# sortmerna/sortmerna

Hardware: NVIDIA H100
Metric: reads/sec (150 bp vs SILVA-8) (higher is better)
Workload: dtype int16x2 (DPX) / u8

## Files before the change

### include/smr_b200.h

```cpp
#ifndef SMR_B200_H
#define SMR_B200_H
#include <stddef.h>
#include <stdint.h>

#ifdef __cplusplus
extern "C" {
#endif

typedef struct smr_ctx smr_ctx;

enum smr_status {
  SMR_OK = 0,
  SMR_ERR_CUDA = 1,
  SMR_ERR_ARG = 2,
  SMR_ERR_INDEX = 3,
  SMR_ERR_UNSUPPORTED = 4,
  SMR_ERR_CAPACITY = 5,
  SMR_ERR_NO_DEVICE = 6
};

typedef struct {
  int32_t match, mismatch, score_N, gap_open, gap_ext;
  int32_t num_seeds, min_lis, edges, edges_is_percent;
  int32_t num_alignments, is_best;
// ... 106 lines not shown
  int32_t out2, sout;
} smr_report_opts;

int smr_format_reports(smr_ctx*, const smr_report_opts* opts, const char* text, uint64_t nbytes, const smr_read_result* results,
                       const smr_aln* alns, const uint32_t* cigar_pool, uint64_t cigar_words, const smr_aln_stats* stats, uint32_t nreads,
                       char* out, uint64_t cap, uint64_t* stream_off);
int smr_format_reports_gz(smr_ctx*, const smr_report_opts* opts, const char* text, uint64_t nbytes, const smr_read_result* results,
                          const smr_aln* alns, const uint32_t* cigar_pool, uint64_t cigar_words, const smr_aln_stats* stats, uint32_t nreads,
                          char* out, uint64_t cap, uint64_t* stream_off);
int smr_gzip(smr_ctx*, const void* in, uint64_t n, void* out, uint64_t cap, uint64_t* out_bytes);
int smr_last_report_timings(const smr_ctx*, double out[3]);

typedef struct {
  double min_id, min_cov;
  int32_t paired_in, paired_out;
} smr_otu_opts;
int smr_otu_begin(smr_ctx*, const smr_otu_opts* opts);
int smr_otu_add(smr_ctx*, const char* text, uint64_t nbytes, const smr_read_result* results, const smr_aln* alns, const smr_aln_stats* stats,
                uint32_t nreads, uint64_t* n_added);
int smr_otu_finish(smr_ctx*, char* out, uint64_t cap, uint64_t counts[3]);
int smr_last_otu_timings(const smr_ctx*, double out[3]);

int smr_last_timings(const smr_ctx*, double out[8]);


int smr_debug_seed_windows(smr_ctx*, uint32_t part_slot, const uint8_t* seq_cat, const uint64_t* seq_off,
                           uint32_t nreads, const uint32_t* win_read, const uint32_t* win_pos, uint32_t nwin,
                           uint32_t* ids, uint32_t cap, uint32_t* counts, uint8_t* zero);
int smr_debug_dpx_peak(smr_ctx*, double* giga_ops_per_s);
int smr_debug_ssw(smr_ctx*, const uint8_t* q_cat, const uint64_t* q_off, const uint8_t* t_cat,
                  const uint64_t* t_off, uint32_t npairs, uint32_t filters, int32_t* out, uint32_t* cigars,
                  uint32_t cigar_cap);

#ifdef __cplusplus
}
#endif
#endif
```

### sortmerna_b200/api.py

```python
from __future__ import annotations

import ctypes as C
import os

import numpy as np

from . import hostio

HERE = os.path.dirname(os.path.abspath(__file__))
LIB_PATH = os.environ.get("SMR_LIB_PATH") or os.path.join(HERE, "libsmr_b200.so")

STATUS = {0: "SMR_OK", 1: "SMR_ERR_CUDA", 2: "SMR_ERR_ARG", 3: "SMR_ERR_INDEX", 4: "SMR_ERR_UNSUPPORTED",
          5: "SMR_ERR_CAPACITY", 6: "SMR_ERR_NO_DEVICE"}

SYMBOLS = ["smr_init", "smr_destroy", "smr_last_error", "smr_device_count", "smr_load_index_part",
           "smr_set_minimal_score", "smr_set_params", "smr_index_info", "smr_align_batch", "smr_upload_batch",
           "smr_run_resident", "smr_download_results", "smr_last_timings", "smr_debug_seed_windows", "smr_debug_ssw",
           "smr_debug_dpx_peak", "smr_set_stats_buffer", "smr_build_index", "smr_upload_fastx", "smr_resident_layout", "smr_pack_kvdb_blobs",
           "smr_set_aln_slots", "smr_aln_slots", "smr_aln_slots_needed", "smr_upload_fastx_gz", "smr_resident_text", "smr_debug_inflate",
           "smr_build_index_device", "smr_debug_index_array", "smr_set_instrumentation", "smr_set_report_refs", "smr_set_report_scoring",
           "smr_format_reports", "smr_last_report_timings", "smr_otu_begin", "smr_otu_add", "smr_otu_finish", "smr_last_otu_timings",
           "smr_format_reports_gz", "smr_gzip"]

CNT_NAMES = ("num_aligned", "num_short", "sw_calls", "sw_cells", "windows", "trie_nodes", "buckets",
             "bucket_entries", "pos_entries", "lis_calls", "dbg_max_read_cycles", "dbg_sum_read_cycles", "dbg_lis_kernel_cycles",
             "cyc_vote", "cyc_order", "cyc_group", "cyc_plan", "cyc_wait", "cyc_replay", "spec_calls", "spec_cells", "spec_pairs", "slow_pairs",
             "sc_wait", "sc_load", "sc_sw", "sc_pub", "rounds_a", "rounds_b", "w1_cyc", "w1_cnt", "dbg_max_read_busy_cycles")
CNT_FIXED = 32


class Params(C.Structure):
    _fields_ = [(n, C.c_int32) for n in (
        "match", "mismatch", "score_N", "gap_open", "gap_ext", "num_seeds", "min_lis", "edges",
        "edges_is_percent", "num_alignments", "is_best", "is_forward", "is_reverse", "is_full_search",
        "minoccur")]


def default_params(**kw) -> Params:
    p = Params(match=2, mismatch=-3, score_N=-3, gap_open=5, gap_ext=2, num_seeds=2, min_lis=2, edges=4,
               edges_is_percent=0, num_alignments=1, is_best=1, is_forward=1, is_reverse=1, is_full_search=0,
               minoccur=0)
    for k, v in kw.items():
        setattr(p, k, v)
    return p

# ... 395 lines not shown
        rc = self.L.smr_otu_finish(self.h, _ptr(buf), C.c_uint64(buf.size), _ptr(counts))
        if rc == 5 and int(counts[0]) > buf.size:
            buf = np.zeros(int(counts[0]) + (int(counts[0]) >> 3), np.uint8)
            rc = self.L.smr_otu_finish(self.h, _ptr(buf), C.c_uint64(buf.size), _ptr(counts))
        self._check(rc, "smr_otu_finish")
        self._otu_buf = buf
        return dict(text=bytes(buf[:int(counts[0])]), total_otu=int(counts[1]), n_yid_ycov=int(counts[2]))

    def otu_timings(self):
        out = np.zeros(3, np.float64)
        self._check(self.L.smr_last_otu_timings(self.h, _ptr(out)), "smr_last_otu_timings")
        return dict(add_h2d_ms=out[0], add_device_ms=out[1], finish_ms=out[2])

    def report_timings(self):
        out = np.zeros(3, np.float64)
        self._check(self.L.smr_last_report_timings(self.h, _ptr(out)), "smr_last_report_timings")
        return dict(h2d_ms=out[0], device_ms=out[1], d2h_ms=out[2])

    def timings(self):
        out = np.zeros(8, np.float64)
        self.L.smr_last_timings(self.h, _ptr(out))
        return dict(total_ms=out[0], seed_ms=out[1], lis_ms=out[2], final_ms=out[3], h2d_ms=out[4], d2h_ms=out[5],
                    launches=int(out[6]), decode_ms=out[7])

    def dpx_peak(self) -> float:
        v = C.c_double(0)
        self._check(self.L.smr_debug_dpx_peak(self.h, C.byref(v)), "smr_debug_dpx_peak")
        return v.value

    def debug_seed_windows(self, part_slot, cat03, off, win_read, win_pos, cap=64, fallback_path=False):
        cat03 = np.ascontiguousarray(cat03, np.uint8)
        off = np.ascontiguousarray(off, np.uint64)
        win_read = np.ascontiguousarray(win_read, np.uint32)
        win_pos = np.ascontiguousarray(win_pos, np.uint32)
        nwin = win_read.size
        ids = np.zeros(nwin * cap, np.uint32)
        counts = np.zeros(nwin, np.uint32)
        zero = np.zeros(nwin, np.uint8)
        rc = self.L.smr_debug_seed_windows(self.h, C.c_uint32(part_slot), _ptr(cat03), _ptr(off), C.c_uint32(off.size - 1),
                                           _ptr(win_read), _ptr(win_pos), C.c_uint32(nwin), _ptr(ids),
                                           C.c_uint32(cap | (0x80000000 if fallback_path else 0)), _ptr(counts), _ptr(zero))
        self._check(rc, "smr_debug_seed_windows")
        return ids.reshape(nwin, cap), counts, zero

    def debug_ssw(self, q_cat, q_off, t_cat, t_off, filters=0, cigar_cap=256):
        q_cat = np.ascontiguousarray(q_cat, np.uint8)
# ... 93 lines not shown
```

### sortmerna_b200/csrc/smr_capi.cu

```cuda
#include "../../include/smr_b200.h"

#include <algorithm>
#include <cmath>
#include <cstdio>
#include <cstdlib>
#include <cstring>
#include <mutex>
#include <string>
#include <thread>
#include <vector>

#include "smr_decode.cuh"
#include "smr_report.cuh"
#include "smr_otu.cuh"
#include "smr_inflate.cuh"
#include "smr_deflate.cuh"
#include "smr_build.h"
#include "smr_build_dev.cuh"
#include "smr_final.cuh"
#include "smr_index.h"

using namespace smr;

namespace {
// ... 42 lines not shown
  uint32_t need_slots = 0;
  uint32_t all_slots = 16;
  uint32_t lis_ctas_per_sm = kLisMinCtas;

  uint32_t nreads = 0; uint64_t total_nt = 0; uint32_t max_len = 0;
  std::vector<uint8_t> h_seq; std::vector<uint64_t> h_off;
  std::vector<uint32_t> off32;
  DevBuf seq04, seq_off, pk03, pk03alt, pk_off, has_n, hit_cnt, flags, state, hit_db, aln_work, out_aln;
  DevBuf hits, cost, bins, scalars, counters, cigar_pool, parts_dev;
  size_t hits_stride = 0; uint32_t cnt_stride = 0;
  DevBuf lis_arena, lis_epochs, lis_queue, lis_done, lis_rows, lis_dbg, final_arena, lane_hits, tb_arena, tb_jobs, fin_list, aln_stats;
  smr_aln_stats* host_stats = nullptr;
  PinBuf h_state, h_flags, h_hitdb, h_outaln, h_stats, h_cigar, h_off32, h_pkoff;
  std::vector<uint64_t> h_coff;
  DevBuf d_text, d_hdroff;
  DevBuf d_cnt, d_scal, d_nl, d_hdr, d_sb, d_rec, d_spos;
  DevBuf cub_tmp;
  DevBuf seed_ctr, d_gz, d_cand, d_res, d_sym, d_win, d_ids, d_off, d_cnt64, d_moff, d_mem, d_poff, d_plen, d_pcrc;
  uint64_t text_bytes = 0;
  uint32_t inf_spans = 0, inf_candidates = 0; double t_inflate = 0;
  bool device_only_reads = false;
  double t_decode = 0;
  uint32_t tb_threads = 0, tb_cap_w = 0, tb_cap_cig = 0; size_t tb_cap_dir = 0, tb_stride = 0;
  uint32_t lis_warps = 0, final_warps = 0;
  size_t lis_stride = 0, final_stride = 0;
  uint32_t hist_cap = 0, cand_cap = 0, pair_cap = 0, row_cap = 0, pall_cap = 0, task_cap = 0, cap_w = 0, cap_cig = 0; size_t cap_dir = 0;
  uint32_t lis_ctas = 0;
  uint32_t lane_hits_cap = 0, lane_hits_warps = 0;
  uint64_t cigar_cap_dev = 0;
  uint32_t scale = 1;
  bool instr = false;
  uint64_t flag_hist[6] = {0, 0, 0, 0, 0, 0};
  struct RptScore { bool set = false; DevBuf ev, bits; };
  std::vector<RptScore> rpt_score;
  DevBuf r_text, r_line, r_recs, r_res, r_aln, r_cig, r_st, r_flags, r_keys, r_keys2, r_vals, r_rows, r_first,
         r_sz, r_off, r_bsz, r_boff, r_fxsz, r_fxoff, r_grp, r_so, r_out;
  double t_rpt[3] = {0, 0, 0};
  DevBuf z_in, z_chunk, z_m, z_freq, z_codes, z_hdr, z_info, z_scratch, z_poff, z_plen, z_crc, z_dst, z_trl, z_out;
  uint64_t parts_gen = 0;
  struct Otu {
    bool active = false; uint64_t gen = 0; double min_id = 0, min_cov = 0;
    std::vector<RptGroup> groups; uint32_t gbits = 0, kbits = 0;
    DevBuf rank, rank_off, grp, key, ent, pool, flag, pos, nsz, noff, vals, skey, sidx, size, off, out, scal;
    uint64_t n = 0, pool_bytes = 0;
    double t[3] = {0, 0, 0};
  } otu;
// ... 155 lines not shown
  pt.d.flookup = p_flookup; pt.d.ftext = p_ftext; pt.d.fid = p_fid; pt.d.pos_off = p_posoff; pt.d.pos = p_pos;
  pt.d.refseq = p_ref; pt.d.ref_off = p_roff;
  pt.n_entries = E; pt.n_ids = nids; pt.n_pos = npos; pt.n_refseq = c04.size();
  return SMR_OK;
}

DevParams to_dev(const smr_params& p) {
  DevParams d;
  d.match = p.match; d.mismatch = p.mismatch; d.score_N = p.score_N; d.gap_open = p.gap_open; d.gap_ext = p.gap_ext;
  d.num_seeds = p.num_seeds; d.min_lis = p.min_lis; d.edges = p.edges; d.edges_is_percent = p.edges_is_percent;
  d.num_alignments = p.num_alignments; d.is_best = p.is_best; d.is_forward = p.is_forward; d.is_reverse = p.is_reverse;
  d.is_full_search = p.is_full_search;
  d.one = 1;
  return d;
}

uint32_t pow2_ge(uint32_t v) { uint32_t p = 1; while (p < v) p <<= 1; return p; }

cudaEvent_t get_event(smr_ctx* ctx, size_t i) {
  while (ctx->ev.size() <= i) { cudaEvent_t e; cudaEventCreate(&e); ctx->ev.push_back(e); }
  return ctx->ev[i];
}

struct Scalars { uint32_t* work_n; uint32_t* lis_next; uint32_t* fin_next; uint32_t* lis_next_b; unsigned long long* cigar_used; uint32_t* fin_jobs; uint32_t* q_head; uint32_t* q_tail; uint32_t* planners_done; };
Scalars scalars_of(smr_ctx* ctx) {
  uint8_t* p = (uint8_t*)ctx->scalars.p;
  return Scalars{(uint32_t*)p, (uint32_t*)(p + 4), (uint32_t*)(p + 8), (uint32_t*)(p + 12), (unsigned long long*)(p + 16), (uint32_t*)(p + 24), (uint32_t*)(p + 128), (uint32_t*)(p + 256), (uint32_t*)(p + 384)};
}

int setup_arenas(smr_ctx* ctx) {
  uint32_t max_nref = 1;
  for (auto& pt : ctx->parts) max_nref = std::max(max_nref, pt.d.nref);
  ctx->hist_cap = max_nref;
  ctx->cand_cap = std::max(64u, max_nref);
  ctx->pair_cap = pow2_ge(4096u * ctx->scale);
  ctx->task_cap = 2 * ctx->pair_cap;
  const uint32_t edges = ctx->prm.edges_is_percent ? (uint32_t)((ctx->prm.edges / 100.0) * (double)ctx->max_len) : (uint32_t)std::max(0, ctx->prm.edges);
  ctx->row_cap = ctx->max_len + 2 * edges + 2 * 64 + 64;
  int occ = 0;
  CK(cudaFuncSetAttribute(lis_kernel<false>, cudaFuncAttributeMaxDynamicSharedMemorySize, kLisSmemBytes));
  CK(cudaFuncSetAttribute(lis_kernel<true>, cudaFuncAttributeMaxDynamicSharedMemorySize, kLisSmemBytes));
  CK(cudaOccupancyMaxActiveBlocksPerMultiprocessor(&occ, lis_kernel<true>, kLisWarpsPerCta * 32, kLisSmemBytes));
  if (occ < 1) { ctx->err = "lis_kernel does not fit on an SM"; return SMR_ERR_CUDA; }
  ctx->lis_ctas = (uint32_t)ctx->sm_count * std::min<uint32_t>(ctx->lis_ctas_per_sm, (uint32_t)occ);
  ctx->lis_warps = ctx->lis_ctas * kPlannerWarps;
  ctx->pall_cap = 32768u * ctx->scale;
  ctx->lis_stride = lis_arena_bytes(ctx->hist_cap, ctx->cand_cap, ctx->pair_cap, ctx->task_cap, ctx->pall_cap);
  const size_t budget = (size_t)16 << 30;
  while (ctx->lis_ctas > 16 && ctx->lis_stride * ctx->lis_warps > budget) { ctx->lis_ctas /= 2; ctx->lis_warps = ctx->lis_ctas * kPlannerWarps; }
  if (int rc = ensure(ctx, ctx->lis_arena, ctx->lis_stride * ctx->lis_warps)) return rc;
  if (int rc = ensure(ctx, ctx->lis_epochs, (size_t)ctx->lis_warps * 4)) return rc;
  if (int rc = ensure(ctx, ctx->lis_queue, (size_t)2 * kQueueCap * sizeof(QSlot) + 64)) return rc;
  if (int rc = ensure(ctx, ctx->lis_done, (size_t)ctx->lis_warps * 4 + 64)) return rc;
  const size_t dbg_bytes = (size_t)(kTlBase + kTlRows * kTlBuckets) * 8;
  if (int rc = ensure(ctx, ctx->lis_dbg, dbg_bytes)) return rc;
  CK(cudaMemsetAsync(ctx->lis_dbg.p, 0, dbg_bytes, ctx->stream));
  if (int rc = ensure(ctx, ctx->lis_rows, (size_t)ctx->lis_ctas * kScorerWarps * 2 * ctx->row_cap * 4)) return rc;
  CK(cudaMemset2DAsync(ctx->lis_arena.p, ctx->lis_stride, 0, lis_arena_zero_bytes(ctx->hist_cap), ctx->lis_warps, ctx->stream));
  CK(cudaMemsetAsync(ctx->lis_epochs.p, 0, (size_t)ctx->lis_warps * 4, ctx->stream));
  ctx->cap_w = 2 * 256 * ctx->scale + 8;
  ctx->cap_cig = 2 * (ctx->max_len + 64) + 16;
  ctx->cap_dir = (size_t)65536 * ctx->scale + (size_t)ctx->max_len * 9 * 3 + 64;
  ctx->final_warps = (uint32_t)ctx->sm_count * kFinalCtasPerSm * kFinalWarpsPerCta;
  ctx->final_stride = final_arena_bytes(ctx->cap_w, ctx->cap_cig, ctx->row_cap, ctx->cap_dir);
  while (ctx->final_warps > 64 && ctx->final_stride * ctx->final_warps > budget) ctx->final_warps /= 2;
  if (int rc = ensure(ctx, ctx->final_arena, ctx->final_stride * ctx->final_warps)) return rc;
  ctx->tb_threads = (uint32_t)ctx->sm_count * 1024u;
  ctx->tb_cap_w = 2 * 32 * ctx->scale + 8;
  ctx->tb_cap_cig = 128 * ctx->scale;
  ctx->tb_cap_dir = (size_t)32768 * ctx->scale;
  ctx->tb_stride = ((size_t)ctx->tb_cap_w * 12 + (size_t)ctx->tb_cap_cig * 4 + ctx->tb_cap_dir + 255) & ~(size_t)255;
  while (ctx->tb_threads > 4096 && ctx->tb_stride * ctx->tb_threads > budget) ctx->tb_threads /= 2;
  if (int rc = ensure(ctx, ctx->tb_arena, ctx->tb_stride * ctx->tb_threads)) return rc;
  ctx->lane_hits_cap = kLaneHitCap * ctx->scale;
  ctx->lane_hits_warps = ctx->scale == 1 ? (uint32_t)ctx->sm_count * kSeedCtasPerSm * kSeedWarpsPerCta : 1024u;
  if (int rc = ensure(ctx, ctx->lane_hits, (size_t)ctx->lane_hits_warps * ctx->lane_hits_cap * 32 * 4)) return rc;
  return SMR_OK;
}

int finish_upload(smr_ctx* ctx, uint32_t nreads, uint64_t w);

int upload_batch_impl(smr_ctx* ctx, const uint8_t* seq_cat, const uint64_t* seq_off, uint32_t nreads, bool keep_host) {
  if (nreads == 0) { ctx->nreads = 0; return SMR_OK; }
  const uint64_t total = seq_off[nreads] - seq_off[0];
  if (total >= 0xF0000000ull) { ctx->err = "batch larger than 2^32 nucleotides: split it"; return SMR_ERR_ARG; }
  cudaEvent_t e0 = get_event(ctx, 0), e1 = get_event(ctx, 1);
  CK(cudaEventRecord(e0, ctx->stream));
  std::vector<uint32_t>& off32 = ctx->off32; off32.resize(nreads + 1);
  { int prc; if ((prc = ensure(ctx, ctx->h_pkoff, (size_t)(nreads + 1) * 4))) return prc; if ((prc = ensure(ctx, ctx->h_off32, (size_t)(nreads + 1) * 4))) return prc; }
  uint32_t* pkoff = (uint32_t*)ctx->h_pkoff.p;
// ... 376 lines not shown
      CK(cudaGetLastError());
      if (ctx->instr) lis_kernel<true><<<ctx->lis_ctas, kLisWarpsPerCta * 32, kLisSmemBytes, ctx->stream>>>(b, dp, lg);
      else lis_kernel<false><<<ctx->lis_ctas, kLisWarpsPerCta * 32, kLisSmemBytes, ctx->stream>>>(b, dp, lg);
      CK(cudaGetLastError());
      CK(cudaEventRecord(s2, ctx->stream));
      spans.push_back({evi - 3, 0});
      ctx->n_launch += 2;
    }
    CK(cudaMemsetAsync(sc.fin_next, 0, 4, ctx->stream));
    CK(cudaMemsetAsync(sc.fin_jobs, 0, 4, ctx->stream));
    cudaEvent_t f0 = get_event(ctx, evi), f1 = get_event(ctx, evi + 1); evi += 2;
    CK(cudaEventRecord(f0, ctx->stream));
    FinalGlobals fg{};
    fg.arena_base = (uint8_t*)ctx->final_arena.p; fg.arena_stride = ctx->final_stride;
    fg.cap_w = ctx->cap_w; fg.cap_cig = ctx->cap_cig; fg.row_cap = ctx->row_cap; fg.cap_dir = ctx->cap_dir;
    fg.parts = (const DevIndex*)ctx->parts_dev.p; fg.aln_work = (const AlnWork*)ctx->aln_work.p; fg.out = (OutAln*)ctx->out_aln.p;
    fg.slots = slots; fg.cigar_pool = (uint32_t*)ctx->cigar_pool.p; fg.cigar_cap = ctx->cigar_cap_dev; fg.cigar_used = sc.cigar_used;
    fg.work_next = sc.fin_next;
    if ((rc = ensure(ctx, ctx->tb_jobs, (size_t)n * slots * sizeof(TraceJob)))) return rc;
    if ((rc = ensure(ctx, ctx->fin_list, (size_t)n * slots * 4))) return rc;
    fg.job_list = (uint32_t*)ctx->fin_list.p; fg.job_count = sc.fin_jobs;
    fg.jobs = (TraceJob*)ctx->tb_jobs.p; fg.tb_arena = (uint8_t*)ctx->tb_arena.p; fg.tb_stride = ctx->tb_stride;
    fg.tb_cap_w = ctx->tb_cap_w; fg.tb_cap_cig = ctx->tb_cap_cig; fg.tb_cap_dir = ctx->tb_cap_dir;
    fg.stats = nullptr;
    if (ctx->host_stats) {
      if ((rc = ensure(ctx, ctx->aln_stats, (size_t)nreads * slots * sizeof(AlnStats)))) return rc;
      fg.stats = (AlnStats*)ctx->aln_stats.p;
    }
    final_jobs_kernel<<<std::min<uint32_t>((n * slots + 255) / 256, (uint32_t)ctx->sm_count * 8), 256, 0, ctx->stream>>>(b, fg);
    CK(cudaGetLastError());
    finalize_kernel<<<ctx->final_warps / kFinalWarpsPerCta, kFinalWarpsPerCta * 32, 0, ctx->stream>>>(b, dp, fg);
    CK(cudaGetLastError());
    traceback_kernel<<<ctx->tb_threads / 128, 128, 0, ctx->stream>>>(b, dp, fg);
    CK(cudaGetLastError());
    ctx->n_launch += 2;
    CK(cudaEventRecord(f1, ctx->stream));
    spans.push_back({evi - 2, 1});
    ctx->n_launch += 1;
  }
  cudaEvent_t ee = get_event(ctx, evi++); CK(cudaEventRecord(ee, ctx->stream));
  CK(cudaStreamSynchronize(ctx->stream));
  float ms = 0;
  cudaEventElapsedTime(&ms, eb, ee); ctx->t_total = ms;
  if (getenv("SMR_VERBOSE")) {
    unsigned long long d[16]; cudaMemcpy(d, ctx->lis_dbg.p, 128, cudaMemcpyDeviceToHost);
    fprintf(stderr, "[smr] slowest read %llu: %.2f ms; cycles vote %llu order %llu group %llu plan %llu wait %llu replay %llu; sw calls %llu, tasks scored %llu, rounds %llu\n", d[10], d[0] / 1.965e6, d[1], d[2], d[3], d[4], d[5], d[6], d[7], d[8], d[9]);
  }
  if (ctx->instr && getenv("SMR_TIMELINE")) {
    std::vector<unsigned long long> tl((size_t)kTlRows * kTlBuckets);
    cudaMemcpy(tl.data(), (const unsigned long long*)ctx->lis_dbg.p + kTlBase, tl.size() * 8, cudaMemcpyDeviceToHost);
    static const char* names[kTlRows] = {"scorer_wait_ns", "scorer_busy_ns", "planner_wait_ns", "planner_vote_group_ns", "reads_done", "planner_alive_ns"};
    for (int r = 0; r < kTlRows; ++r) {
      int last = 0; for (int k = 0; k < kTlBuckets; ++k) if (tl[(size_t)r * kTlBuckets + k]) last = k + 1;
      fprintf(stderr, "[smr timeline] %s", names[r]);
      for (int k = 0; k < last; ++k) fprintf(stderr, " %llu", tl[(size_t)r * kTlBuckets + k]);
      fprintf(stderr, "\n");
// ... 20 lines not shown
  const uint32_t slots = slots_of(ctx);
  cudaEvent_t e0 = get_event(ctx, 0), e1 = get_event(ctx, 1);
  CK(cudaEventRecord(e0, ctx->stream));
  int prc;
  if ((prc = ensure(ctx, ctx->h_state, (size_t)n * sizeof(ReadState)))) return prc;
  if ((prc = ensure(ctx, ctx->h_flags, (size_t)n * 4))) return prc;
  if ((prc = ensure(ctx, ctx->h_hitdb, (size_t)n * 2))) return prc;
  if ((prc = ensure(ctx, ctx->h_outaln, (size_t)n * slots * sizeof(OutAln)))) return prc;
  const ReadState* st = (const ReadState*)ctx->h_state.p; const uint32_t* fl = (const uint32_t*)ctx->h_flags.p;
  const uint16_t* hdb = (const uint16_t*)ctx->h_hitdb.p; const OutAln* oa = (const OutAln*)ctx->h_outaln.p;
  const AlnStats* ast = nullptr;
  if (ctx->host_stats) {
    if ((prc = ensure(ctx, ctx->h_stats, (size_t)n * slots * sizeof(AlnStats)))) return prc;
    ast = (const AlnStats*)ctx->h_stats.p;
    CK(cudaMemcpyAsync(ctx->h_stats.p, ctx->aln_stats.p, (size_t)n * slots * sizeof(AlnStats), cudaMemcpyDeviceToHost, ctx->stream));
  }
  unsigned long long used = 0;
  std::vector<unsigned long long> cnt(dcCount + 64);
  CK(cudaMemcpyAsync(ctx->h_state.p, ctx->state.p, (size_t)n * sizeof(ReadState), cudaMemcpyDeviceToHost, ctx->stream));
  CK(cudaMemcpyAsync(ctx->h_flags.p, ctx->flags.p, (size_t)n * 4, cudaMemcpyDeviceToHost, ctx->stream));
  CK(cudaMemcpyAsync(ctx->h_hitdb.p, ctx->hit_db.p, (size_t)n * 2, cudaMemcpyDeviceToHost, ctx->stream));
  CK(cudaMemcpyAsync(ctx->h_outaln.p, ctx->out_aln.p, (size_t)n * slots * sizeof(OutAln), cudaMemcpyDeviceToHost, ctx->stream));
  CK(cudaMemcpyAsync(&used, scalars_of(ctx).cigar_used, 8, cudaMemcpyDeviceToHost, ctx->stream));
  CK(cudaMemcpyAsync(cnt.data(), ctx->counters.p, cnt.size() * 8, cudaMemcpyDeviceToHost, ctx->stream));
  CK(cudaStreamSynchronize(ctx->stream));
  used = std::min<unsigned long long>(used, ctx->cigar_cap_dev);
  if ((prc = ensure(ctx, ctx->h_cigar, (size_t)used * 4 + 16))) return prc;
  const uint32_t* cig = (const uint32_t*)ctx->h_cigar.p;
  if (used) CK(cudaMemcpyAsync(ctx->h_cigar.p, ctx->cigar_pool.p, used * 4, cudaMemcpyDeviceToHost, ctx->stream));
  CK(cudaEventRecord(e1, ctx->stream));
  CK(cudaStreamSynchronize(ctx->stream));
  float ms = 0; cudaEventElapsedTime(&ms, e0, e1); ctx->t_d2h = ms;
  int rc = SMR_OK;
  std::vector<uint64_t>& coff = ctx->h_coff; coff.resize((size_t)n + 1);
  uint64_t run = out.cigar_used;
  uint32_t need_slots = 0;
  for (uint32_t r = 0; r < n; ++r) {
    coff[r] = run;
    if (fl[r] & kErrTrace) { ctx->err = "trace back error (ssw.c:707 is fatal in the reference too)"; rc = SMR_ERR_INDEX; }
    if (fl[r] & kOvfSlots) { need_slots = std::max(need_slots, st[r].n_align); continue; }
    if (fl[r]) { flagged.push_back(r); for (int bit = 0; bit < 6; ++bit) if (fl[r] & (1u << bit)) ctx->flag_hist[bit]++; continue; }
    const ReadState& s = st[r];
    for (uint32_t k = 0; k < slots && k < s.n_align; ++k) run += oa[(size_t)r * slots + k].cigar_len;
    if (s.is_hit && out.counters) {
      if (out.n_counters > SMR_CNT_NUM_ALIGNED) out.counters[SMR_CNT_NUM_ALIGNED]++;
      const uint32_t ci = SMR_CNT_FIXED + hdb[r];
      if (hdb[r] != 0xFFFF && ci < out.n_counters) out.counters[ci]++;
    }
  }
// ... 47 lines not shown
  }
  return rc;
}

int align_impl(smr_ctx* ctx, const uint8_t* seq_cat, const uint64_t* seq_off, uint32_t nreads, HostOut& out, const uint32_t* map, int depth) {
  int rc = upload_batch_impl(ctx, seq_cat, seq_off, nreads, false);
  if (rc) return rc;
  const double h2d = ctx->t_h2d;
  if ((rc = run_impl(ctx))) return rc;
  std::vector<uint32_t> flagged;
  if ((rc = download_impl(ctx, out, flagged, map))) return rc;
  ctx->t_h2d = h2d;
  if (flagged.empty()) return SMR_OK;
  if (getenv("SMR_VERBOSE")) fprintf(stderr, "[smr] %zu reads overflowed their scratch at scale %u: retrying with scale %u (causes so far: lane %llu region %llu pairs %llu trace %llu cigar %llu err %llu)\n", flagged.size(), ctx->scale, ctx->scale * 8,
      (unsigned long long)ctx->flag_hist[0], (unsigned long long)ctx->flag_hist[1], (unsigned long long)ctx->flag_hist[2], (unsigned long long)ctx->flag_hist[3], (unsigned long long)ctx->flag_hist[4], (unsigned long long)ctx->flag_hist[5]);
  if (depth >= 3) { ctx->err = "scratch overflow persists after 3 retries (" + std::to_string(flagged.size()) + " reads)"; return SMR_ERR_CAPACITY; }
  std::vector<uint8_t> sseq; std::vector<uint64_t> soff(1, 0); std::vector<uint32_t> smap;
  for (uint32_t r : flagged) {
    sseq.insert(sseq.end(), seq_cat + seq_off[r], seq_cat + seq_off[r + 1]);
    soff.push_back(sseq.size());
    smap.push_back(map ? map[r] : r);
  }
  const uint32_t old_scale = ctx->scale;
  const double tt = ctx->t_total, ts = ctx->t_seed, tl = ctx->t_lis, tf = ctx->t_final, td = ctx->t_d2h; const uint64_t nl = ctx->n_launch;
  ctx->scale = old_scale * 8;
  rc = align_impl(ctx, sseq.data(), soff.data(), (uint32_t)flagged.size(), out, smap.data(), depth + 1);
  ctx->scale = old_scale;
  ctx->t_total += tt; ctx->t_seed += ts; ctx->t_lis += tl; ctx->t_final += tf; ctx->t_d2h += td; ctx->t_h2d += h2d; ctx->n_launch += nl;
  return rc;
}

template <class T>
int upload_async(smr_ctx* ctx, DevBuf& b, const T* src, size_t n) {
  int rc;
  if ((rc = ensure(ctx, b, n * sizeof(T) + 16))) return rc;
  if (n) CK(cudaMemcpyAsync(b.p, src, n * sizeof(T), cudaMemcpyHostToDevice, ctx->stream));
  return SMR_OK;
}

int rpt_error(smr_ctx* ctx, uint32_t e) {
  ctx->err = e & kRptErrLen ? "an alignment's readlen or read_end1 disagrees with the length of its read in the text"
           : e & kRptErrGroup ? "an alignment names an (index, part) that is not loaded"
           : e & kRptErrRef ? "an alignment's ref_num is beyond the reference names of its part"
           : e & kRptErrQual ? "reads text: a FASTQ record without its quality line" : "an alignment's CIGAR lies outside cigar_words";
  return SMR_ERR_ARG;
}

int rpt_prologue(smr_ctx* ctx, const char* text, uint64_t nbytes, const smr_read_result* results, const smr_aln* alns, const uint32_t* cigar,
                 uint64_t cigar_words, const smr_aln_stats* stats, uint32_t nreads, const std::vector<RptGroup>& hg, cudaEvent_t e1, RptArgs& a) {
  const uint32_t slots = slots_of(ctx), G = (uint32_t)hg.size();
  const uint64_t N = (uint64_t)nreads * slots;
// ... 413 lines not shown
  catch (const std::bad_alloc&) { if (ctx) (ctx)->err = "out of host memory"; return SMR_ERR_CAPACITY; } \
  catch (const std::exception& ex) { if (ctx) (ctx)->err = std::string("internal error: ") + ex.what(); return SMR_ERR_CUDA; }

int smr_device_count(void) {
  int n = 0;
  if (cudaGetDeviceCount(&n) != cudaSuccess) return 0;
  return n;
}

int smr_init(int device, smr_ctx** out) {
  if (!out) return SMR_ERR_ARG;
  *out = nullptr;
  int n = 0;
  if (cudaGetDeviceCount(&n) != cudaSuccess || n == 0 || device < 0 || device >= n) return SMR_ERR_NO_DEVICE;
  smr_ctx* ctx = new smr_ctx();
  ctx->device = device;
  if (cudaSetDevice(device) != cudaSuccess) { delete ctx; return SMR_ERR_NO_DEVICE; }
  cudaDeviceProp prop;
  if (cudaGetDeviceProperties(&prop, device) != cudaSuccess) { delete ctx; return SMR_ERR_NO_DEVICE; }
  ctx->sm_count = prop.multiProcessorCount;
  if (cudaStreamCreateWithFlags(&ctx->stream, cudaStreamNonBlocking) != cudaSuccess) { delete ctx; return SMR_ERR_CUDA; }
  if (const char* e = getenv("SMR_CHUNK_READS")) { const long v = atol(e); if (v >= 32 && v <= (1l << 22)) ctx->chunk_reads = (uint32_t)v; }
  if (const char* e = getenv("SMR_INSTR")) ctx->instr = atoi(e) != 0;
  if (const char* e = getenv("SMR_LIS_CTAS_PER_SM")) { const int v = atoi(e); if (v >= 1 && v <= 16) ctx->lis_ctas_per_sm = (uint32_t)v; }
  *out = ctx;
  return SMR_OK;
}

void smr_destroy(smr_ctx* ctx) {
  if (!ctx) return;
  cudaSetDevice(ctx->device);
  for (cudaEvent_t e : ctx->ev) cudaEventDestroy(e);
  if (ctx->stream) cudaStreamDestroy(ctx->stream);
  delete ctx;
}

const char* smr_last_error(const smr_ctx* ctx) { return ctx ? ctx->err.c_str() : "null context"; }

int smr_load_index_part(smr_ctx* ctx, uint32_t index_num, uint32_t part, const void* kmer_file, size_t kmer_bytes,
                        const void* bursttrie_file, size_t bursttrie_bytes, const void* pos_file, size_t pos_bytes,
                        const uint8_t* refseq_cat, const uint64_t* ref_off, uint32_t nref, uint32_t lnwin, uint32_t minimal_score,
                        const uint32_t skiplengths[3]) {
  if (!ctx || !kmer_file || !bursttrie_file || !pos_file || !refseq_cat || !ref_off || !skiplengths) return SMR_ERR_ARG;
  if (skiplengths[0] == 0 || skiplengths[1] == 0 || skiplengths[2] == 0) { ctx->err = "skiplengths must be positive"; return SMR_ERR_ARG; }
  CK(cudaSetDevice(ctx->device));
  FlatIndex fx;
// ... 347 lines not shown
  }
  int rc;
  if ((rc = ensure(ctx, ctx->z_in, n + 64))) return rc;
  CK(cudaMemsetAsync((uint8_t*)ctx->z_in.p + n, 0, 64, ctx->stream));
  CK(cudaMemcpyAsync(ctx->z_in.p, in, n, cudaMemcpyHostToDevice, ctx->stream));
  CK(cudaEventRecord(e1, ctx->stream));
  uint64_t so[2];
  rc = gzip_streams(ctx, (const uint8_t*)ctx->z_in.p, {0}, {n}, (char*)out, cap, so, e2, e3);
  *out_bytes = so[1];
  if (rc) return rc;
  float ms = 0;
  cudaEventElapsedTime(&ms, e0, e1); ctx->t_rpt[0] = ms;
  cudaEventElapsedTime(&ms, e1, e2); ctx->t_rpt[1] = ms;
  cudaEventElapsedTime(&ms, e2, e3); ctx->t_rpt[2] = ms;
  return SMR_OK;
} SMR_CATCH(ctx)

int smr_last_report_timings(const smr_ctx* ctx, double out[3]) {
  if (!ctx || !out) return SMR_ERR_ARG;
  for (int k = 0; k < 3; ++k) out[k] = ctx->t_rpt[k];
  return SMR_OK;
}

int smr_last_timings(const smr_ctx* ctx, double out[8]) {
  if (!ctx || !out) return SMR_ERR_ARG;
  out[0] = ctx->t_total; out[1] = ctx->t_seed; out[2] = ctx->t_lis; out[3] = ctx->t_final; out[4] = ctx->t_h2d; out[5] = ctx->t_d2h;
  out[6] = (double)ctx->n_launch; out[7] = ctx->t_decode;
  return SMR_OK;
}

int smr_debug_dpx_peak(smr_ctx* ctx, double* giga_ops_per_s) {
  if (!ctx || !giga_ops_per_s) return SMR_ERR_ARG;
  CK(cudaSetDevice(ctx->device));
  DevBuf d;
  CK(d.alloc(64));
  const int iters = 1 << 14, ctas = ctx->sm_count * 8, thr = 256;
  cudaEvent_t e0 = get_event(ctx, 0), e1 = get_event(ctx, 1);
  double best = 0;
  for (int rep = 0; rep < 4; ++rep) {
    CK(cudaEventRecord(e0, ctx->stream));
    dpx_peak_kernel<<<ctas, thr, 0, ctx->stream>>>((int32_t*)d.p, iters, -2, -1000000);
    CK(cudaGetLastError());
    CK(cudaEventRecord(e1, ctx->stream));
    CK(cudaStreamSynchronize(ctx->stream));
    float ms = 0; cudaEventElapsedTime(&ms, e0, e1);
    const double ops = (double)ctas * thr * iters * 8.0;
// ... 96 lines not shown
```

### sortmerna_b200/csrc/smr_final.cuh

```cuda
#pragma once
#include "smr_lis.cuh"

namespace smr {

struct OutAln {
  uint32_t cigar_off, cigar_len, ref_num;
  int32_t ref_begin1, ref_end1, read_begin1, read_end1;
  uint32_t readlen;
  uint16_t score1, part, index_num;
  uint8_t strand, pad;
};

struct TraceJob {
  uint32_t valid;
  uint32_t idx_slot, ref_num, ref_off;
  int32_t q_start, q_step;
  int32_t rl, ql, score, band;
};

struct AlnStats { uint32_t n_miss, n_gap, n_match, n_match_denovo; };

struct FinalGlobals {
  uint8_t* arena_base; size_t arena_stride;
  uint32_t cap_w, cap_cig, row_cap; size_t cap_dir;
  const DevIndex* parts;
  const AlnWork* aln_work; OutAln* out; uint32_t slots;
  uint32_t* cigar_pool; unsigned long long cigar_cap; unsigned long long* cigar_used;
  uint32_t* work_next;
  uint32_t* job_list; uint32_t* job_count;
  struct TraceJob* jobs;
  uint8_t* tb_arena; size_t tb_stride; uint32_t tb_cap_w, tb_cap_cig; size_t tb_cap_dir;
  AlnStats* stats;
};
__host__ __device__ inline size_t final_arena_bytes(uint32_t cap_w, uint32_t cap_cig, uint32_t row_cap, size_t cap_dir) {
  size_t b = (size_t)cap_w * 12 + (size_t)cap_cig * 4 + (size_t)row_cap * 8 + cap_dir;
  return (b + 255) & ~(size_t)255;
}

constexpr int kFinalWarpsPerCta = 4;
#ifndef SMR_FINAL_MIN_CTAS
#define SMR_FINAL_MIN_CTAS 6
#endif
constexpr int kFinalCtasPerSm = SMR_FINAL_MIN_CTAS;

__global__ void __launch_bounds__(256)
final_jobs_kernel(DevBatch b, FinalGlobals g) {
  const uint32_t total = b.nreads * g.slots;
  const unsigned lane = lane_id();
  for (uint32_t w0 = (blockIdx.x * blockDim.x + threadIdx.x) & ~31u; w0 < total; w0 += gridDim.x * blockDim.x) {
    const uint32_t wi = w0 + lane;
    bool live = false;
    if (wi < total) {
      const uint32_t r = b.r0 + wi / g.slots, k = wi % g.slots;
      live = k < b.state[r].n_align && !b.flags[r];
// ... 99 lines not shown
    if (lane == 0) j0 = atomicAdd(g.work_next, 2u);
    j0 = __shfl_sync(kFull, j0, 0);
    if (j0 >= njobs) break;
    const bool two = j0 + 1 < njobs;
    const uint32_t w0 = g.job_list[j0], w1 = two ? g.job_list[j0 + 1] : 0u;
    uint2 ef = make_uint2(kPairNoHit, kPairNoHit), er = ef;
    bool p0, p1;
    {
      const PairLoc L0 = final_loc(b, g, w0), L1 = two ? final_loc(b, g, w1) : no_loc();
      p0 = final_packed(L0, sc); p1 = two && final_packed(L1, sc);
      if (p0 || p1) ef = sw_pair_locate(p0 ? L0 : no_loc(), p1 ? L1 : no_loc(), sc, S.prof, S.win[0], S.win[1]);
    }
    const bool r0 = p0 && ef.x != kPairNoHit, r1 = p1 && ef.y != kPairNoHit;
    if (r0 || r1) {
      const PairLoc R0 = r0 ? reverse_loc(final_loc(b, g, w0), ef.x) : no_loc(), R1 = r1 ? reverse_loc(final_loc(b, g, w1), ef.y) : no_loc();
      er = sw_pair_locate(R0, R1, sc, S.prof, S.win[0], S.win[1]);
    }
    final_finish(b, sc, g, S, rowH, rowF, j0, w0, p0, ef.x, er.x);
    if (two) final_finish(b, sc, g, S, rowH, rowF, j0 + 1, w1, p1, ef.y, er.y);
    __syncwarp();
  }
}

__global__ void __launch_bounds__(128)
traceback_kernel(DevBatch b, DevParams prm, FinalGlobals g) {
  const uint32_t tid = blockIdx.x * blockDim.x + threadIdx.x, nthreads = gridDim.x * blockDim.x;
  const uint32_t lane = threadIdx.x & 31;
  uint8_t* p = g.tb_arena + (size_t)(tid >> 5) * g.tb_stride * 32;
  TraceArena A;
  A.cap_w = g.tb_cap_w; A.cap_cig = g.tb_cap_cig; A.cap_dir = g.tb_cap_dir; A.stride = 32;
  A.hb = (int32_t*)p + lane; p += (size_t)g.tb_cap_w * 4 * 32;
  A.eb = (int32_t*)p + lane; p += (size_t)g.tb_cap_w * 4 * 32;
  A.hc = (int32_t*)p + lane; p += (size_t)g.tb_cap_w * 4 * 32;
  A.cig = (uint32_t*)p + lane; p += (size_t)g.tb_cap_cig * 4 * 32;
  A.dir = (int8_t*)p + lane;
  const SwScore sc{prm.match, prm.mismatch, prm.score_N, prm.gap_open, prm.gap_ext, prm.one};
  const uint32_t njobs = *g.job_count;
  for (uint32_t ji = tid; ji < njobs; ji += nthreads) {
    const TraceJob j = g.jobs[ji];
    if (!j.valid) continue;
    const uint32_t wi = g.job_list[ji];
    const uint32_t r = b.r0 + wi / g.slots, k = wi % g.slots;
    const DevIndex& ix = g.parts[j.idx_slot];
    const SeqView t{ix.refseq + ix.ref_off[j.ref_num], (int32_t)j.ref_off, 1, false};
    const SeqView q{b.seq04 + b.seq_off[r], j.q_start, j.q_step, j.q_step < 0};
    for (uint32_t i = 0; i < g.tb_cap_w; ++i) { A.hb[i * 32] = 0; A.eb[i * 32] = 0; A.hc[i * 32] = 0; }
    const int32_t nc = banded_traceback_lane(t, q, j.rl, j.ql, j.score, sc, j.band, A);
    if (nc < 0) { atomicOr(&b.flags[r], nc == -1 ? kOvfTrace : kErrTrace); continue; }
    const unsigned long long off = atomicAdd(g.cigar_used, (unsigned long long)nc);
    if (off + (unsigned long long)nc > g.cigar_cap) { atomicOr(&b.flags[r], kOvfCigar); continue; }
    for (int32_t i = 0; i < nc; ++i) g.cigar_pool[off + i] = A.cig[(size_t)(nc - 1 - i) * 32];
    OutAln* o = g.out + (size_t)r * g.slots + k;
    o->cigar_off = (uint32_t)off; o->cigar_len = (uint32_t)nc;
    if (g.stats) {
      const SeqView qd{b.seq04 + b.seq_off[r], o->read_begin1, 1, false};
      uint32_t miss = 0, gap = 0, match = 0, match_d = 0;
      int32_t x = 0, y = 0;
      for (int32_t i = nc - 1; i >= 0; --i) {
        const uint32_t c = A.cig[(size_t)i * 32], op = c & 0xFu, ln = c >> 4;
        if (op == 0) {
          for (uint32_t u = 0; u < ln; ++u, ++x, ++y) {
            const uint32_t tc = t.at(x);
            if (tc != q.at(y)) ++miss; else ++match;
            match_d += tc == qd.at(y);
          }
        }
        else if (op == 1) { y += (int32_t)ln; gap += ln; }
        else { x += (int32_t)ln; gap += ln; }
      }
      g.stats[(size_t)r * g.slots + k] = AlnStats{miss, gap, match, match_d};
    }
  }
}

__global__ void __launch_bounds__(kFinalWarpsPerCta * 32)
ssw_debug_kernel(const uint8_t* qcat, const uint32_t* qoff, const uint8_t* tcat, const uint32_t* toff, uint32_t npairs, uint32_t filters,
                 DevParams prm, int32_t* out, uint32_t* cigars, uint32_t cigar_cap, FinalGlobals g) {
  __shared__ FinalSmem s_fin[kFinalWarpsPerCta];
  const unsigned lane = lane_id();
  const uint32_t warp = blockIdx.x * kFinalWarpsPerCta + (threadIdx.x >> 5), nwarps = gridDim.x * kFinalWarpsPerCta;
  int32_t *rowH, *rowF;
  TraceArena A = final_arena(g, warp, rowH, rowF);
  FinalSmem& S = s_fin[threadIdx.x >> 5];
  uint8_t* s_ref = S.win[0]; int32_t* s_prof = (int32_t*)S.prof;
  const SwScore sc{prm.match, prm.mismatch, prm.score_N, prm.gap_open, prm.gap_ext, prm.one};
  for (uint32_t k0 = 2 * warp; k0 < npairs; k0 += 2 * nwarps) {
    PairLoc L[2], RL[2];
    SwEnd fe[2], re[2];
#pragma unroll 1
    for (uint32_t h = 0; h < 2; ++h) {
      L[h] = no_loc(); RL[h] = no_loc();
      const uint32_t k = k0 + h;
      if (k >= npairs) break;
      const int32_t m = (int32_t)(qoff[k + 1] - qoff[k]), n = (int32_t)(toff[k + 1] - toff[k]);
      const SeqView q{qcat + qoff[k], 0, 1, false}, t{tcat + toff[k], 0, 1, false};
// ... 54 lines not shown
```

Measured before the change: 4.916 million.

## Run banded traceback DP rows in shared memory with packed direction nibbles

Result: no change. 4.957 million (median of 6 runs) (+0.8%).

```diff
diff --git a/include/smr_b200.h b/include/smr_b200.h
--- a/include/smr_b200.h
+++ b/include/smr_b200.h
@@ -152,6 +152,7 @@
 int smr_last_otu_timings(const smr_ctx*, double out[3]);
 
 int smr_last_timings(const smr_ctx*, double out[8]);
+int smr_last_trace_wide(const smr_ctx*, uint64_t* n);
 
 
 int smr_debug_seed_windows(smr_ctx*, uint32_t part_slot, const uint8_t* seq_cat, const uint64_t* seq_off,
diff --git a/sortmerna_b200/api.py b/sortmerna_b200/api.py
--- a/sortmerna_b200/api.py
+++ b/sortmerna_b200/api.py
@@ -20,7 +20,7 @@
            "smr_set_aln_slots", "smr_aln_slots", "smr_aln_slots_needed", "smr_upload_fastx_gz", "smr_resident_text", "smr_debug_inflate",
            "smr_build_index_device", "smr_debug_index_array", "smr_set_instrumentation", "smr_set_report_refs", "smr_set_report_scoring",
            "smr_format_reports", "smr_last_report_timings", "smr_otu_begin", "smr_otu_add", "smr_otu_finish", "smr_last_otu_timings",
-           "smr_format_reports_gz", "smr_gzip"]
+           "smr_format_reports_gz", "smr_gzip", "smr_last_trace_wide"]
 
 CNT_NAMES = ("num_aligned", "num_short", "sw_calls", "sw_cells", "windows", "trie_nodes", "buckets",
              "bucket_entries", "pos_entries", "lis_calls", "dbg_max_read_cycles", "dbg_sum_read_cycles", "dbg_lis_kernel_cycles",
@@ -462,6 +462,11 @@
         self.L.smr_last_timings(self.h, _ptr(out))
         return dict(total_ms=out[0], seed_ms=out[1], lis_ms=out[2], final_ms=out[3], h2d_ms=out[4], d2h_ms=out[5],
                     launches=int(out[6]), decode_ms=out[7])
+
+    def trace_wide(self) -> int:
+        v = C.c_uint64(0)
+        self._check(self.L.smr_last_trace_wide(self.h, C.byref(v)), "smr_last_trace_wide")
+        return v.value
 
     def dpx_peak(self) -> float:
         v = C.c_double(0)
diff --git a/sortmerna_b200/csrc/smr_capi.cu b/sortmerna_b200/csrc/smr_capi.cu
--- a/sortmerna_b200/csrc/smr_capi.cu
+++ b/sortmerna_b200/csrc/smr_capi.cu
@@ -88,6 +88,8 @@
   bool device_only_reads = false;
   double t_decode = 0;
   uint32_t tb_threads = 0, tb_cap_w = 0, tb_cap_cig = 0; size_t tb_cap_dir = 0, tb_stride = 0;
+  uint32_t tb_rows_w = kTraceRowW;
+  uint64_t n_trace_wide = 0;
   uint32_t lis_warps = 0, final_warps = 0;
   size_t lis_stride = 0, final_stride = 0;
   uint32_t hist_cap = 0, cand_cap = 0, pair_cap = 0, row_cap = 0, pall_cap = 0, task_cap = 0, cap_w = 0, cap_cig = 0; size_t cap_dir = 0;
@@ -289,10 +291,10 @@
   return ctx->ev[i];
 }
 
-struct Scalars { uint32_t* work_n; uint32_t* lis_next; uint32_t* fin_next; uint32_t* lis_next_b; unsigned long long* cigar_used; uint32_t* fin_jobs; uint32_t* q_head; uint32_t* q_tail; uint32_t* planners_done; };
+struct Scalars { uint32_t* work_n; uint32_t* lis_next; uint32_t* fin_next; uint32_t* lis_next_b; unsigned long long* cigar_used; uint32_t* fin_jobs; unsigned long long* tb_wide; uint32_t* q_head; uint32_t* q_tail; uint32_t* planners_done; };
 Scalars scalars_of(smr_ctx* ctx) {
   uint8_t* p = (uint8_t*)ctx->scalars.p;
-  return Scalars{(uint32_t*)p, (uint32_t*)(p + 4), (uint32_t*)(p + 8), (uint32_t*)(p + 12), (unsigned long long*)(p + 16), (uint32_t*)(p + 24), (uint32_t*)(p + 128), (uint32_t*)(p + 256), (uint32_t*)(p + 384)};
+  return Scalars{(uint32_t*)p, (uint32_t*)(p + 4), (uint32_t*)(p + 8), (uint32_t*)(p + 12), (unsigned long long*)(p + 16), (uint32_t*)(p + 24), (unsigned long long*)(p + 32), (uint32_t*)(p + 128), (uint32_t*)(p + 256), (uint32_t*)(p + 384)};
 }
 
 int setup_arenas(smr_ctx* ctx) {
@@ -332,7 +334,7 @@
   ctx->final_stride = final_arena_bytes(ctx->cap_w, ctx->cap_cig, ctx->row_cap, ctx->cap_dir);
   while (ctx->final_warps > 64 && ctx->final_stride * ctx->final_warps > budget) ctx->final_warps /= 2;
   if (int rc = ensure(ctx, ctx->final_arena, ctx->final_stride * ctx->final_warps)) return rc;
-  ctx->tb_threads = (uint32_t)ctx->sm_count * 1024u;
+  ctx->tb_threads = (uint32_t)ctx->sm_count * kTraceCtasPerSm * kTraceThreads;
   ctx->tb_cap_w = 2 * 32 * ctx->scale + 8;
   ctx->tb_cap_cig = 128 * ctx->scale;
   ctx->tb_cap_dir = (size_t)32768 * ctx->scale;
@@ -755,6 +757,7 @@
     fg.job_list = (uint32_t*)ctx->fin_list.p; fg.job_count = sc.fin_jobs;
     fg.jobs = (TraceJob*)ctx->tb_jobs.p; fg.tb_arena = (uint8_t*)ctx->tb_arena.p; fg.tb_stride = ctx->tb_stride;
     fg.tb_cap_w = ctx->tb_cap_w; fg.tb_cap_cig = ctx->tb_cap_cig; fg.tb_cap_dir = ctx->tb_cap_dir;
+    fg.tb_rows_w = ctx->tb_rows_w; fg.tb_wide = sc.tb_wide;
     fg.stats = nullptr;
     if (ctx->host_stats) {
       if ((rc = ensure(ctx, ctx->aln_stats, (size_t)nreads * slots * sizeof(AlnStats)))) return rc;
@@ -764,7 +767,7 @@
     CK(cudaGetLastError());
     finalize_kernel<<<ctx->final_warps / kFinalWarpsPerCta, kFinalWarpsPerCta * 32, 0, ctx->stream>>>(b, dp, fg);
     CK(cudaGetLastError());
-    traceback_kernel<<<ctx->tb_threads / 128, 128, 0, ctx->stream>>>(b, dp, fg);
+    traceback_kernel<<<ctx->tb_threads / kTraceThreads, kTraceThreads, 0, ctx->stream>>>(b, dp, fg);
     CK(cudaGetLastError());
     ctx->n_launch += 2;
     CK(cudaEventRecord(f1, ctx->stream));
@@ -831,9 +834,12 @@
   CK(cudaMemcpyAsync(ctx->h_hitdb.p, ctx->hit_db.p, (size_t)n * 2, cudaMemcpyDeviceToHost, ctx->stream));
   CK(cudaMemcpyAsync(ctx->h_outaln.p, ctx->out_aln.p, (size_t)n * slots * sizeof(OutAln), cudaMemcpyDeviceToHost, ctx->stream));
   CK(cudaMemcpyAsync(&used, scalars_of(ctx).cigar_used, 8, cudaMemcpyDeviceToHost, ctx->stream));
+  unsigned long long wide = 0;
+  CK(cudaMemcpyAsync(&wide, scalars_of(ctx).tb_wide, 8, cudaMemcpyDeviceToHost, ctx->stream));
   CK(cudaMemcpyAsync(cnt.data(), ctx->counters.p, cnt.size() * 8, cudaMemcpyDeviceToHost, ctx->stream));
   CK(cudaStreamSynchronize(ctx->stream));
   used = std::min<unsigned long long>(used, ctx->cigar_cap_dev);
+  ctx->n_trace_wide = wide;
   if ((prc = ensure(ctx, ctx->h_cigar, (size_t)used * 4 + 16))) return prc;
   const uint32_t* cig = (const uint32_t*)ctx->h_cigar.p;
   if (used) CK(cudaMemcpyAsync(ctx->h_cigar.p, ctx->cigar_pool.p, used * 4, cudaMemcpyDeviceToHost, ctx->stream));
@@ -927,11 +933,12 @@
     smap.push_back(map ? map[r] : r);
   }
   const uint32_t old_scale = ctx->scale;
+  const uint64_t nw = ctx->n_trace_wide;
   const double tt = ctx->t_total, ts = ctx->t_seed, tl = ctx->t_lis, tf = ctx->t_final, td = ctx->t_d2h; const uint64_t nl = ctx->n_launch;
   ctx->scale = old_scale * 8;
   rc = align_impl(ctx, sseq.data(), soff.data(), (uint32_t)flagged.size(), out, smap.data(), depth + 1);
   ctx->scale = old_scale;
-  ctx->t_total += tt; ctx->t_seed += ts; ctx->t_lis += tl; ctx->t_final += tf; ctx->t_d2h += td; ctx->t_h2d += h2d; ctx->n_launch += nl;
+  ctx->t_total += tt; ctx->t_seed += ts; ctx->t_lis += tl; ctx->t_final += tf; ctx->t_d2h += td; ctx->t_h2d += h2d; ctx->n_launch += nl; ctx->n_trace_wide += nw;
   return rc;
 }
 
@@ -1391,6 +1398,7 @@
   if (cudaStreamCreateWithFlags(&ctx->stream, cudaStreamNonBlocking) != cudaSuccess) { delete ctx; return SMR_ERR_CUDA; }
   if (const char* e = getenv("SMR_CHUNK_READS")) { const long v = atol(e); if (v >= 32 && v <= (1l << 22)) ctx->chunk_reads = (uint32_t)v; }
   if (const char* e = getenv("SMR_INSTR")) ctx->instr = atoi(e) != 0;
+  if (const char* e = getenv("SMR_TRACE_GLOBAL")) if (atoi(e) != 0) ctx->tb_rows_w = 0;
   if (const char* e = getenv("SMR_LIS_CTAS_PER_SM")) { const int v = atoi(e); if (v >= 1 && v <= 16) ctx->lis_ctas_per_sm = (uint32_t)v; }
   *out = ctx;
   return SMR_OK;
@@ -1784,6 +1792,12 @@
   return SMR_OK;
 }
 
+int smr_last_trace_wide(const smr_ctx* ctx, uint64_t* n) {
+  if (!ctx || !n) return SMR_ERR_ARG;
+  *n = ctx->n_trace_wide;
+  return SMR_OK;
+}
+
 int smr_last_timings(const smr_ctx* ctx, double out[8]) {
   if (!ctx || !out) return SMR_ERR_ARG;
   out[0] = ctx->t_total; out[1] = ctx->t_seed; out[2] = ctx->t_lis; out[3] = ctx->t_final; out[4] = ctx->t_h2d; out[5] = ctx->t_d2h;
diff --git a/sortmerna_b200/csrc/smr_final.cuh b/sortmerna_b200/csrc/smr_final.cuh
--- a/sortmerna_b200/csrc/smr_final.cuh
+++ b/sortmerna_b200/csrc/smr_final.cuh
@@ -1,5 +1,6 @@
 #pragma once
 #include "smr_lis.cuh"
+#include "smr_trace.h"
 
 namespace smr {
 
@@ -30,6 +31,8 @@
   uint32_t* job_list; uint32_t* job_count;
   struct TraceJob* jobs;
   uint8_t* tb_arena; size_t tb_stride; uint32_t tb_cap_w, tb_cap_cig; size_t tb_cap_dir;
+  uint32_t tb_rows_w;
+  unsigned long long* tb_wide;
   AlnStats* stats;
 };
 __host__ __device__ inline size_t final_arena_bytes(uint32_t cap_w, uint32_t cap_cig, uint32_t row_cap, size_t cap_dir) {
@@ -175,8 +178,10 @@
   }
 }
 
-__global__ void __launch_bounds__(128)
+constexpr uint32_t kTraceThreads = 128, kTraceCtasPerSm = 8;
+__global__ void __launch_bounds__(kTraceThreads, kTraceCtasPerSm)
 traceback_kernel(DevBatch b, DevParams prm, FinalGlobals g) {
+  __shared__ int32_t s_rows[2 * kTraceRowW * kTraceThreads];
   const uint32_t tid = blockIdx.x * blockDim.x + threadIdx.x, nthreads = gridDim.x * blockDim.x;
   const uint32_t lane = threadIdx.x & 31;
   uint8_t* p = g.tb_arena + (size_t)(tid >> 5) * g.tb_stride * 32;
@@ -187,8 +192,12 @@
   A.hc = (int32_t*)p + lane; p += (size_t)g.tb_cap_w * 4 * 32;
   A.cig = (uint32_t*)p + lane; p += (size_t)g.tb_cap_cig * 4 * 32;
   A.dir = (int8_t*)p + lane;
+  uint32_t* dir_words = (uint32_t*)p + lane;
+  int32_t* s_hb = s_rows + threadIdx.x;
+  int32_t* s_eb = s_rows + kTraceRowW * kTraceThreads + threadIdx.x;
   const SwScore sc{prm.match, prm.mismatch, prm.score_N, prm.gap_open, prm.gap_ext, prm.one};
   const uint32_t njobs = *g.job_count;
+  uint32_t n_wide = 0;
   for (uint32_t ji = tid; ji < njobs; ji += nthreads) {
     const TraceJob j = g.jobs[ji];
     if (!j.valid) continue;
@@ -197,8 +206,15 @@
     const DevIndex& ix = g.parts[j.idx_slot];
     const SeqView t{ix.refseq + ix.ref_off[j.ref_num], (int32_t)j.ref_off, 1, false};
     const SeqView q{b.seq04 + b.seq_off[r], j.q_start, j.q_step, j.q_step < 0};
-    for (uint32_t i = 0; i < g.tb_cap_w; ++i) { A.hb[i * 32] = 0; A.eb[i * 32] = 0; A.hc[i * 32] = 0; }
-    const int32_t nc = banded_traceback_lane(t, q, j.rl, j.ql, j.score, sc, j.band, A);
+    int32_t nc = kTraceWide;
+    if ((uint32_t)j.band * 2 + 4 <= g.tb_rows_w)
+      nc = banded_trace_rows(t, q, j.rl, j.ql, j.score, sc, j.band, s_hb, s_eb, kTraceThreads, g.tb_rows_w, dir_words, 32, A.cap_dir,
+                             A.cig, 32, A.cap_cig);
+    if (nc == kTraceWide) {
+      ++n_wide;
+      for (uint32_t i = 0; i < g.tb_cap_w; ++i) { A.hb[i * 32] = 0; A.eb[i * 32] = 0; A.hc[i * 32] = 0; }
+      nc = banded_traceback_lane(t, q, j.rl, j.ql, j.score, sc, j.band, A);
+    }
     if (nc < 0) { atomicOr(&b.flags[r], nc == -1 ? kOvfTrace : kErrTrace); continue; }
     const unsigned long long off = atomicAdd(g.cigar_used, (unsigned long long)nc);
     if (off + (unsigned long long)nc > g.cigar_cap) { atomicOr(&b.flags[r], kOvfCigar); continue; }
@@ -224,6 +240,8 @@
       g.stats[(size_t)r * g.slots + k] = AlnStats{miss, gap, match, match_d};
     }
   }
+  n_wide = __reduce_add_sync(kFull, n_wide);
+  if (lane == 0 && n_wide) atomicAdd(g.tb_wide, (unsigned long long)n_wide);
 }
 
 __global__ void __launch_bounds__(kFinalWarpsPerCta * 32)
diff --git a/sortmerna_b200/csrc/smr_trace.h b/sortmerna_b200/csrc/smr_trace.h
--- /dev/null
+++ b/sortmerna_b200/csrc/smr_trace.h
@@ -0,0 +1,105 @@
+#pragma once
+#include <stddef.h>
+#include <stdint.h>
+
+#if defined(__CUDACC__)
+#define SMR_TR_HD __host__ __device__ __forceinline__
+#else
+#define SMR_TR_HD inline
+#endif
+
+namespace smr {
+
+constexpr uint32_t kTraceRowW = 24;
+constexpr int32_t kTraceWide = -3;
+
+SMR_TR_HD int32_t trace_max(int32_t a, int32_t b) { return a > b ? a : b; }
+SMR_TR_HD int32_t trace_min(int32_t a, int32_t b) { return a < b ? a : b; }
+
+#if defined(__CUDACC__)
+#pragma nv_exec_check_disable
+#endif
+template <class Ref, class Qry, class Score>
+SMR_TR_HD int32_t banded_trace_rows(const Ref& t, const Qry& q, const int32_t refLen, const int32_t readLen, const int32_t score,
+                                    const Score& sc, int32_t band_width, int32_t* hb, int32_t* eb, const uint32_t rs, const uint32_t cap_w,
+                                    uint32_t* dir, const uint32_t ds, const size_t cap_dir, uint32_t* cig, const uint32_t cs,
+                                    const uint32_t cap_cig) {
+  for (uint32_t k = 0; k < cap_w; ++k) { hb[k * rs] = 0; eb[k * rs] = 0; }
+  int32_t maxv = 0, width = 0, width_d = 0, words = 0;
+  do {
+    width = band_width * 2 + 3; width_d = band_width * 2 + 1; words = (width_d + 7) >> 3;
+    if ((uint32_t)(width + 1) > cap_w) return kTraceWide;
+    if ((size_t)width_d * readLen * 3 + 8 > cap_dir) return -1;
+    for (int32_t k = 1; k < width - 1; ++k) hb[k * rs] = 0;
+    for (int32_t i = 0; i < readLen; ++i) {
+      const int32_t x = trace_max(0, i - band_width), end = trace_min(refLen - 1, i + band_width);
+      const int32_t n = end - x + 1;
+      const int32_t edge = end + 1 < width - 1 ? end + 1 : width - 1;
+      const int32_t s = i > band_width ? 1 : 0;
+      hb[0] = 0; eb[0] = 0; hb[edge * rs] = 0; eb[edge * rs] = 0;
+      const uint32_t qi = q.at(i);
+      uint32_t* drow = dir + (size_t)i * words * ds;
+      int32_t f = 0, hleft = 0;
+      int32_t hdg = hb[s * rs], hup = hb[(1 + s) * rs], eup = eb[(1 + s) * rs];
+      uint32_t wd = 0;
+      int32_t k = 0;
+      for (int32_t u = 1; u <= n; ++u) {
+        const int32_t hu = hup, eu = eup;
+        hup = hb[(u + 1 + s) * rs]; eup = eb[(u + 1 + s) * rs];
+        const uint32_t tj = t.at(x + u - 1);
+        int32_t t1 = i == 0 ? -sc.go : hu - sc.go;
+        int32_t t2 = i == 0 ? -sc.ge : eu - sc.ge;
+        const int32_t ev = t1 > t2 ? t1 : t2;
+        const uint32_t ce = t1 > t2 ? 1u : 0u;
+        eb[u * rs] = ev;
+        t1 = hleft - sc.go; t2 = f - sc.ge;
+        f = t1 > t2 ? t1 : t2;
+        const uint32_t cf = t1 > t2 ? 2u : 0u;
+        const int32_t e1 = ev > 0 ? ev : 0, f1 = f > 0 ? f : 0;
+        t1 = e1 > f1 ? e1 : f1;
+        const int32_t sv = (tj >= 4u || qi >= 4u) ? sc.sN : (tj == qi ? sc.match : sc.mismatch);
+        t2 = hdg + sv;
+        hdg = hu;
+        const int32_t hv = t1 > t2 ? t1 : t2;
+        hb[u * rs] = hv; hleft = hv;
+        if (hv > maxv) maxv = hv;
+        const uint32_t ch = (t1 <= t2) ? 4u : (e1 > f1 ? 8u : 12u);
+        wd |= (ce | cf | ch) << (((u - 1) & 7) * 4);
+        if (((u - 1) & 7) == 7) { drow[(k++) * ds] = wd; wd = 0; }
+      }
+      for (; k < words; ++k) { drow[k * ds] = wd; wd = 0; }
+    }
+    band_width *= 2;
+  } while (maxv < score);
+  band_width /= 2;
+  int32_t i = readLen - 1, j = refLen - 1, run = 0, cur_op = 0, op = 0, which = 2;
+  uint32_t l = 0;
+  while (i > 0) {
+    int32_t r = i, c = j - trace_max(0, i - band_width);
+    while (c < 0) { c += width_d; --r; }
+    while (c >= width_d) { c -= width_d; ++r; }
+    if (r < 0 || r >= readLen) return -2;
+    const uint32_t nib = (dir[((size_t)r * words + (c >> 3)) * ds] >> ((c & 7) * 4)) & 15u;
+    const uint32_t ce = 2u + (nib & 1u), cf = 4u + ((nib >> 1) & 1u), ch = nib >> 2;
+    const uint32_t code = ch == 0 ? 0u : which == 0 ? ce : which == 1 ? cf : ch == 1 ? 1u : ch == 2 ? ce : cf;
+    switch (code) {
+      case 1: --i; --j; which = 2; op = 0; break;
+      case 2: --i; which = 0; op = 1; break;
+      case 3: --i; which = 2; op = 1; break;
+      case 4: --j; which = 1; op = 2; break;
+      case 5: --j; which = 2; op = 2; break;
+      default: return -2;
+    }
+    if (op == cur_op) ++run;
+    else {
+      if (l >= cap_cig) return -1;
+      cig[(l++) * cs] = (uint32_t)run << 4 | (uint32_t)cur_op; cur_op = op; run = 1;
+    }
+  }
+  if (l + 2 > cap_cig) return -1;
+  if (op == 0) cig[(l++) * cs] = (uint32_t)(run + 1) << 4;
+  else { cig[(l++) * cs] = (uint32_t)run << 4 | (uint32_t)op; cig[(l++) * cs] = 16u; }
+  return (int32_t)l;
+}
+
+}
```
